# irfanICMLL/structure_knowledge_distillation

Hardware: AMD Instinct MI355X
Metric: distillation-step images/sec @512x512 (Pi+Pa+Ho) (higher is better)
Workload: dtype f32; 1 GPU; BASELINE configs[2]: ResNet18-PSPNet student + frozen ResNet101-PSPNet teacher, Pi+Pa+Ho (SAGAN D, spectral norm, WGAN-GP), batch 8 per GPU, 512x512, 19 classes; global_batch=8, parallelism=dp1

## Files before the change

structure_knowledge_distillation_amd/csrc/conv1x1.hip:

```cpp
#include <stdio.h>
#include <stdlib.h>

#include "conv_split_dev.hpp"

namespace skd {
namespace {

constexpr int kProMaxK = 512;

template <int TM>
struct Staging {
  float4 a[TM / kRPP], b[kRB];
};
struct ProParams {
  float4 pm, pi, pg, pb;
};

template <bool PRO, int TM>
__device__ __forceinline__ void stage_load(Staging<TM> &s, const float *__restrict__ X, const float *__restrict__ Wt, int k0,
                                           int gkq, const int64_t (&arow)[TM / kRPP], int64_t wrow0, int K) {
  const float *xa = X + k0 + gkq, *wb = Wt + k0 + gkq;
#pragma unroll
  for (int h = 0; h < TM / kRPP; ++h) s.a[h] = *reinterpret_cast<const float4 *>(xa + arow[h]);
#pragma unroll
  for (int h = 0; h < kRB; ++h) s.b[h] = *reinterpret_cast<const float4 *>(wb + wrow0 + (int64_t)(kRPP * h) * K);
}

__device__ __forceinline__ float pro_one(float x, float m, float is, float g, float b) {
  const float z = __builtin_fmaf((x - m) * is, g, b);
  return z < 0.f ? 0.f : z;
}

template <bool PRO, int TM>
__device__ __forceinline__ void stage_store(const Staging<TM> s, uint4 *stage, int srow, const float *ptab, int K, int kq) {
  constexpr int kRA = TM / kRPP;
  uint2 *sa = reinterpret_cast<uint2 *>(stage) + srow, *sb = reinterpret_cast<uint2 *>(stage + kOperandChunks) + srow;
  if (PRO) {
    ProParams pp;
    pp.pm = *reinterpret_cast<const float4 *>(ptab + kq);
    pp.pi = *reinterpret_cast<const float4 *>(ptab + K + kq);
    pp.pg = *reinterpret_cast<const float4 *>(ptab + 2 * K + kq);
    pp.pb = *reinterpret_cast<const float4 *>(ptab + 3 * K + kq);
#pragma unroll
    for (int h = 0; h < kRA; ++h) {
      float4 v = s.a[h];
      v.x = pro_one(v.x, pp.pm.x, pp.pi.x, pp.pg.x, pp.pb.x);
      v.y = pro_one(v.y, pp.pm.y, pp.pi.y, pp.pg.y, pp.pb.y);
      v.z = pro_one(v.z, pp.pm.z, pp.pi.z, pp.pg.z, pp.pb.z);
      v.w = pro_one(v.w, pp.pm.w, pp.pi.w, pp.pg.w, pp.pb.w);
      split_store(v, sa + 2 * kRPP * h);
    }
  } else {
#pragma unroll
    for (int h = 0; h < kRA; ++h) split_store(s.a[h], sa + 2 * kRPP * h);
  }
#pragma unroll
  for (int h = 0; h < kRB; ++h) split_store(s.b[h], sb + 2 * kRPP * h);
}

template <int TM, int ACT, bool HAS_RES, bool PRO, bool NT>
__device__ __forceinline__ void conv1x1_tile(const float *__restrict__ X, const float *__restrict__ Wt, const float *__restrict__ R,
                                             float *__restrict__ Y, const float *__restrict__ mean, const float *__restrict__ var,
                                             const float *__restrict__ weight, const float *__restrict__ bias,
                                             const float *__restrict__ ppack, float eps, float slope, int64_t M, int K, int N,
                                             int64_t m0, int n0, uint4 *lds) {
  constexpr int WM = TM / 64, kRA = TM / kRPP;
  f32x16 acc[WM][2];
#pragma unroll
  for (int i = 0; i < WM; ++i)
#pragma unroll
    for (int j = 0; j < 2; ++j)
#pragma unroll
      for (int q = 0; q < 16; ++q) acc[i][j][q] = 0.f;
  const int nk = K / kBK;
  const int gt = threadIdx.x, grow = gt / kQK, gkq = (gt % kQK) * 4;
  const int srow = plane_slot(grow, gkq);
  int64_t arow[kRA];
#pragma unroll
  for (int h = 0; h < kRA; ++h) {
    const int64_t m = m0 + grow + kRPP * h;
    arow[h] = (m > M - 1 ? M - 1 : m) * K;
  }
  const int64_t wrow0 = (int64_t)(n0 + grow) * K;
  float *ptab = reinterpret_cast<float *>(lds + 2 * kStageChunks);
  if (PRO) {
    for (int i = gt * 4; i < 4 * K; i += kThreads * 4) *reinterpret_cast<float4 *>(ptab + i) = *reinterpret_cast<const float4 *>(ppack + i);
    __syncthreads();
  }
  Staging<TM> st;
  stage_load<PRO, TM>(st, X, Wt, 0, gkq, arow, wrow0, K);
  stage_store<PRO, TM>(st, lds, srow, ptab, K, gkq);
  __syncthreads();
  int stage = 0;
  for (int kt = 0; kt < nk; ++kt) {
    const bool more = kt + 1 < nk;
    if (more) stage_load<PRO, TM>(st, X, Wt, (kt + 1) * kBK, gkq, arow, wrow0, K);
    tile_mma<TM>(lds + stage * kStageChunks, acc);
    if (more) stage_store<PRO, TM>(st, lds + (stage ^ 1) * kStageChunks, srow, ptab, K, (kt + 1) * kBK + gkq);
    __syncthreads();
    stage ^= 1;
  }
  const int lane = threadIdx.x & (kWave - 1), wid = threadIdx.x / kWave;
  const int wi = (wid >> 1) * (TM / 2), wj = (wid & 1) * 64;
  const bool full = m0 + TM <= M;
#pragma unroll
  for (int bj = 0; bj < 2; ++bj) {
    const int col = n0 + wj + bj * 32 + (lane & 31);
    const float mu = mean[col], is = inv_std_of(var[col], eps);
    const float ga = weight != nullptr ? fabsf(weight[col]) + eps : 1.f;
    const float be = bias != nullptr ? bias[col] : 0.f;
#pragma unroll
    for (int bi = 0; bi < WM; ++bi) {
      const int64_t row0 = m0 + wi + bi * 32;
      if (full)
        store_block<ACT, HAS_RES, true, NT>(acc[bi][bj], R, Y, row0, col, M, N, mu, is, ga, be, slope);
      else
        store_block<ACT, HAS_RES, false, NT>(acc[bi][bj], R, Y, row0, col, M, N, mu, is, ga, be, slope);
    }
  }
}

struct Geometry {
  int tiles_n, ct, pm;
  int64_t p_full, panels, grid;
  bool nt;
};
inline bool conv1x1_geometry(int64_t M, int K, int N, int cus, Geometry &g) {
  g.tiles_n = N / kTN;
  const int64_t tiles_m = cdiv(M, kTM);
  const int64_t tile_bytes = (int64_t)kTN * K * sizeof(float);
  g.ct = (int)((1 << 20) / tile_bytes);
  g.pm = (int)((2 << 20) / tile_bytes);
  if (g.ct < 1) g.ct = 1;
  if (g.pm < 1) g.pm = 1;
  g.nt = g.ct < g.tiles_n;
  if (!g.nt) { g.ct = g.tiles_n; g.pm = 1; }
  while (g.tiles_n % g.ct) --g.ct;
  g.p_full = g.panels = tiles_m;
  const int64_t slots = (int64_t)kMinWG * cus;
  const int64_t tiles = tiles_m * g.tiles_n;
  if (slots > 0 && tiles > slots && tiles % slots != 0) {
    g.p_full = (tiles / slots) * slots / g.tiles_n / 8 * 8;
    const int64_t rest_rows = M - g.p_full * kTM;
    g.panels = g.p_full + cdiv(rest_rows, kTM / 2);
  }
  const int64_t panels_per_xcd = cdiv(cdiv(g.panels, 8), g.pm) * g.pm;
  g.grid = panels_per_xcd * 8 * g.tiles_n;
  return g.grid <= 2147483647;
}

struct TileOf {
  int64_t m0;
  int rows, n0;
};
__host__ __device__ __forceinline__ TileOf conv1x1_tile_of(unsigned block, int64_t M, int tiles_n, int pm, int ct, int p_full) {
  const int xcd = block & 7, j = block >> 3;
  const int per_group = pm * tiles_n;
  const int group = j / per_group, r = j - group * per_group;
  const int per_chunk = pm * ct;
  const int chunk = r / per_chunk, r2 = r - chunk * per_chunk;
  const int pl = r2 / ct;
  const int tn = chunk * ct + (r2 - pl * ct);
  const int64_t tm = ((int64_t)group * pm + pl) * 8 + xcd;
  if (tn >= tiles_n) return TileOf{0, 0, 0};
  if (tm < p_full) {
    const int64_t m0 = tm * kTM;
    if (m0 >= M) return TileOf{0, 0, 0};
    return TileOf{m0, kTM, tn * kTN};
  }
  const int64_t m0 = (int64_t)p_full * kTM + (tm - p_full) * (kTM / 2);
  if (m0 >= M) return TileOf{0, 0, 0};
  return TileOf{m0, kTM / 2, tn * kTN};
}

template <int ACT, bool HAS_RES, bool PRO, bool NT>
__global__ __launch_bounds__(kThreads, kMinWG) void conv1x1_abn_kernel(
    const float *__restrict__ X, const float *__restrict__ Wt, const float *__restrict__ R, float *__restrict__ Y,
    const float *__restrict__ mean, const float *__restrict__ var, const float *__restrict__ weight,
    const float *__restrict__ bias, const float *__restrict__ ppack, float eps, float slope, int64_t M, int K, int N,
    int tiles_n, int pm, int ct, int p_full) {
  extern __shared__ __attribute__((aligned(16))) uint4 lds[];
  const TileOf t = conv1x1_tile_of(blockIdx.x, M, tiles_n, pm, ct, p_full);
  if (t.rows == kTM)
    conv1x1_tile<kTM, ACT, HAS_RES, PRO, NT>(X, Wt, R, Y, mean, var, weight, bias, ppack, eps, slope, M, K, N, t.m0, t.n0, lds);
  else if (t.rows == kTM / 2)
    conv1x1_tile<kTM / 2, ACT, HAS_RES, PRO, NT>(X, Wt, R, Y, mean, var, weight, bias, ppack, eps, slope, M, K, N, t.m0, t.n0, lds);
}

__global__ void pack_eval_params_kernel(int K, const float *__restrict__ mean, const float *__restrict__ var,
                                        const float *__restrict__ weight, const float *__restrict__ bias, float eps,
                                        float *__restrict__ pack) {
  const int k = blockIdx.x * blockDim.x + threadIdx.x;
  if (k >= K) return;
  pack[k] = mean[k];
  pack[K + k] = inv_std_of(var[k], eps);
  pack[2 * (int64_t)K + k] = weight != nullptr ? fabsf(weight[k]) + eps : 1.f;
  pack[3 * (int64_t)K + k] = bias != nullptr ? bias[k] : 0.f;
}

template <int ACT, bool HAS_RES, bool PRO, bool NT = false>
static int launch(const float *X, const float *Wt, const float *R, float *Y, const float *mean, const float *var,
                  const float *weight, const float *bias, const float *ppack, float eps, float slope, int64_t M, int K, int N,
                  hipStream_t st) {
  static PerDeviceFlag ready;
  bool *rdy = ready.get();
  if (rdy == nullptr) return 0;
  if (!*rdy) {
    if (hipFuncSetAttribute(reinterpret_cast<const void *>(conv1x1_abn_kernel<ACT, HAS_RES, PRO, NT>),
                            hipFuncAttributeMaxDynamicSharedMemorySize, (int)(kConvLds + sizeof(float) * 4 * kProMaxK)) != hipSuccess) return 0;
    *rdy = true;
  }
  const size_t lds_bytes = kConvLds + (PRO ? sizeof(float) * 4 * (size_t)K : 0);
  Geometry g;
  if (!conv1x1_geometry(M, K, N, cu_count(st), g)) return 0;
  if (g.nt && !NT) return launch<ACT, HAS_RES, PRO, true>(X, Wt, R, Y, mean, var, weight, bias, ppack, eps, slope, M, K, N, st);
  conv1x1_abn_kernel<ACT, HAS_RES, PRO, NT><<<dim3((unsigned)g.grid), dim3(kThreads), lds_bytes, st>>>(
      X, Wt, R, Y, mean, var, weight, bias, ppack, eps, slope, M, K, N, g.tiles_n, g.pm, g.ct, (int)g.p_full);
  return ok();
}

}
}

using namespace skd;

extern "C" {

int skd_conv1x1_abn_supported(int64_t M, int K, int N) { return M > 0 && K > 0 && N > 0 && K % kBK == 0 && N % kTN == 0; }

int skd_conv1x1_abn_geometry(int64_t M, int K, int N, int cus, int64_t *out) {
  Geometry g;
  if (!skd_conv1x1_abn_supported(M, K, N) || cus < 0 || !out || !conv1x1_geometry(M, K, N, cus, g)) return 0;
  out[0] = g.tiles_n; out[1] = g.ct; out[2] = g.pm; out[3] = g.p_full; out[4] = g.panels; out[5] = g.grid; out[6] = g.nt;
  return 1;
}

int skd_conv1x1_abn_tile_of(int64_t M, int K, int N, int cus, int64_t block, int64_t count, int64_t *out) {
  Geometry g;
  if (!skd_conv1x1_abn_supported(M, K, N) || cus < 0 || !out || !conv1x1_geometry(M, K, N, cus, g)) return 0;
  if (block < 0 || count < 0 || block > g.grid || count > g.grid - block) return 0;
  for (int64_t i = 0; i < count; ++i) {
    const TileOf t = conv1x1_tile_of((unsigned)(block + i), M, g.tiles_n, g.pm, g.ct, (int)g.p_full);
    out[3 * i] = t.m0; out[3 * i + 1] = t.rows; out[3 * i + 2] = t.n0;
  }
  return 1;
}

static int conv1x1_dispatch(int64_t M, int K, int N, const float *x, const float *w, const float *residual, float *out,
                            const float *mean, const float *var, const float *weight, const float *bias, const float *ppack,
                            float eps, int activation, float slope, skd_stream_t stream) {
  if (!skd_conv1x1_abn_supported(M, K, N) || !x || !w || !out || !mean || !var) return 0;
  if ((reinterpret_cast<uintptr_t>(x) | reinterpret_cast<uintptr_t>(w) | reinterpret_cast<uintptr_t>(ppack)) & 15) return 0;
  hipStream_t st = as_stream(stream);
#define SKD_C11(A)                                                                                                        \
  if (ppack != nullptr)                                                                                                   \
    return residual ? launch<A, true, true>(x, w, residual, out, mean, var, weight, bias, ppack, eps, slope, M, K, N, st)   \
                    : launch<A, false, true>(x, w, residual, out, mean, var, weight, bias, ppack, eps, slope, M, K, N, st); \
  return residual ? launch<A, true, false>(x, w, residual, out, mean, var, weight, bias, nullptr, eps, slope, M, K, N, st) \
                  : launch<A, false, false>(x, w, residual, out, mean, var, weight, bias, nullptr, eps, slope, M, K, N, st)
  switch (activation) {
    case SKD_ACT_NONE: SKD_C11(SKD_ACT_NONE);
    case SKD_ACT_RELU: SKD_C11(SKD_ACT_RELU);
    case SKD_ACT_LEAKY_RELU: SKD_C11(SKD_ACT_LEAKY_RELU);
    default: return 0;
  }
#undef SKD_C11
}

int skd_conv1x1_abn_nhwc(int64_t M, int K, int N, const float *x, const float *w, const float *residual, float *out,
                         const float *mean, const float *var, const float *weight, const float *bias, float eps,
                         int activation, float slope, skd_stream_t stream) {
  return conv1x1_dispatch(M, K, N, x, w, residual, out, mean, var, weight, bias, nullptr, eps, activation, slope, stream);
}

int skd_abn_pack_eval_params(int K, const float *mean, const float *var, const float *weight, const float *bias, float eps,
                             float *pack, skd_stream_t stream) {
  if (K <= 0 || !mean || !var || !pack) return 0;
  pack_eval_params_kernel<<<dim3((unsigned)cdiv(K, 256)), dim3(256), 0, as_stream(stream)>>>(K, mean, var, weight, bias, eps, pack);
  return ok();
}

int skd_conv1x1_abn_pro_nhwc(int64_t M, int K, int N, const float *x, const float *w, const float *residual, float *out,
                             const float *mean, const float *var, const float *weight, const float *bias, float eps,
                             const float *ppack, int activation, float slope, skd_stream_t stream) {
  if (!ppack || K > kProMaxK) return 0;
  return conv1x1_dispatch(M, K, N, x, w, residual, out, mean, var, weight, bias, ppack, eps, activation, slope, stream);
}

}
```

structure_knowledge_distillation_amd/csrc/conv3x3.hip:

```cpp
#include "conv_split_dev.hpp"

namespace skd {
namespace {

constexpr int kTileChunks = kOperandChunks;
constexpr int kBChunksPerThread = kTileChunks / kThreads;

template <int TM>
struct Staging3 {
  float4 a[TM / kRPP];
  uint4 b[kBChunksPerThread];
};

struct TapCursor {
  int tap, c0;
  int64_t shift;
};

__device__ __forceinline__ int64_t tap_shift(int tap, int W, int dil, int Cin) {
  const int ty = tap / 3, tx = tap - 3 * ty;
  return ((int64_t)(ty - 1) * W + (tx - 1)) * dil * Cin;
}

template <int TM>
__device__ __forceinline__ void stage_load3(Staging3<TM> &s, const float *__restrict__ X, const uint4 *__restrict__ bsrc,
                                            const TapCursor &cur, const int64_t (&abase)[TM / kRPP], const unsigned (&mask)[TM / kRPP]) {
#pragma unroll
  for (int h = 0; h < TM / kRPP; ++h) {
    s.a[h] = make_float4(0.f, 0.f, 0.f, 0.f);
    if ((mask[h] >> cur.tap) & 1u) s.a[h] = *reinterpret_cast<const float4 *>(X + abase[h] + cur.shift + cur.c0);
  }
#pragma unroll
  for (int p = 0; p < kBChunksPerThread; ++p) s.b[p] = bsrc[p * kPlaneChunks];
}

template <int TM>
__device__ __forceinline__ void stage_store3(const Staging3<TM> s, uint4 *stage, int srow) {
  uint2 *sa = reinterpret_cast<uint2 *>(stage) + srow;
#pragma unroll
  for (int h = 0; h < TM / kRPP; ++h) split_store(s.a[h], sa + 2 * kRPP * h);
  uint4 *sb = stage + kOperandChunks + threadIdx.x;
#pragma unroll
  for (int p = 0; p < kBChunksPerThread; ++p) sb[p * kPlaneChunks] = s.b[p];
}

template <int TM, int ACT>
__device__ __forceinline__ void conv3x3_tile(const float *__restrict__ X, const uint4 *__restrict__ Bp, float *__restrict__ Y,
                                             const float *__restrict__ cbias, const float *__restrict__ mean,
                                             const float *__restrict__ var, const float *__restrict__ weight,
                                             const float *__restrict__ bias, float eps, float slope, int64_t M, int H, int W,
                                             int Cin, int N, int dil, int64_t m0, int tn, uint4 *lds) {
  constexpr int WM = TM / 64, kRA = TM / kRPP;
  f32x16 acc[WM][2], low[WM][2];
#pragma unroll
  for (int i = 0; i < WM; ++i)
#pragma unroll
    for (int j = 0; j < 2; ++j)
#pragma unroll
      for (int q = 0; q < 16; ++q) acc[i][j][q] = low[i][j][q] = 0.f;
  const int nk = 9 * (Cin / kBK);
  const int gt = threadIdx.x, grow = gt / kQK, gkq = (gt % kQK) * 4;
  const int srow = plane_slot(grow, gkq);
  int64_t abase[kRA];
  unsigned mask[kRA];
  const int64_t hw = (int64_t)H * W;
#pragma unroll
  for (int h = 0; h < kRA; ++h) {
    const int64_t m = m0 + grow + kRPP * h;
    const bool live = m < M;
    const int64_t mm = live ? m : 0;
    const int pix = (int)(mm % hw);
    const int py = pix / W, px = pix - py * W;
    unsigned bits = 0;
#pragma unroll
    for (int tap = 0; tap < 9; ++tap) {
      const int64_t y = py + (int64_t)(tap / 3 - 1) * dil, x = px + (int64_t)(tap % 3 - 1) * dil;
      if (live && y >= 0 && y < H && x >= 0 && x < W) bits |= 1u << tap;
    }
    mask[h] = bits;
    abase[h] = mm * Cin + gkq;
  }
  const uint4 *bsrc = Bp + (int64_t)tn * nk * kTileChunks + gt;
  TapCursor cur = {0, 0, tap_shift(0, W, dil, Cin)};
  Staging3<TM> st;
  stage_load3<TM>(st, X, bsrc, cur, abase, mask);
  stage_store3<TM>(st, lds, srow);
  __syncthreads();
  int stage = 0;
  for (int kt = 0; kt < nk; ++kt) {
    const bool more = kt + 1 < nk;
    if (more) {
      cur.c0 += kBK;
      if (cur.c0 == Cin) {
        cur.c0 = 0;
        ++cur.tap;
        cur.shift = tap_shift(cur.tap, W, dil, Cin);
      }
      stage_load3<TM>(st, X, bsrc + (int64_t)(kt + 1) * kTileChunks, cur, abase, mask);
    }
    tile_mma<TM>(lds + stage * kStageChunks, low, acc);
    if (more) stage_store3<TM>(st, lds + (stage ^ 1) * kStageChunks, srow);
    __syncthreads();
    stage ^= 1;
  }
  const int lane = threadIdx.x & (kWave - 1), wid = threadIdx.x / kWave;
  const int wi = (wid >> 1) * (TM / 2), wj = (wid & 1) * 64;
  const bool full = m0 + TM <= M;
#pragma unroll
  for (int bj = 0; bj < 2; ++bj) {
    const int col = tn * kTN + wj + bj * 32 + (lane & 31);
    const bool bn = mean != nullptr;
    const float mu = bn ? mean[col] : 0.f, is = bn ? inv_std_of(var[col], eps) : 1.f;
    const float ga = bn && weight != nullptr ? fabsf(weight[col]) + eps : 1.f;
    const float be = bn && bias != nullptr ? bias[col] : 0.f;
    const float cb = cbias != nullptr ? cbias[col] : 0.f;
#pragma unroll
    for (int bi = 0; bi < WM; ++bi) {
#pragma unroll
      for (int q = 0; q < 16; ++q) acc[bi][bj][q] += low[bi][bj][q];
      if (cbias != nullptr) {
#pragma unroll
        for (int q = 0; q < 16; ++q) acc[bi][bj][q] += cb;
      }
      const int64_t row0 = m0 + wi + bi * 32;
      if (full)
        store_block<ACT, false, true, false>(acc[bi][bj], nullptr, Y, row0, col, M, N, mu, is, ga, be, slope);
      else
        store_block<ACT, false, false, false>(acc[bi][bj], nullptr, Y, row0, col, M, N, mu, is, ga, be, slope);
    }
  }
}

template <int ACT, bool TALL>
__global__ __launch_bounds__(kThreads, TALL ? 2 : kMinWG) __attribute__((amdgpu_waves_per_eu(TALL ? 2 : kMinWG, TALL ? 2 : kMinWG)))
void conv3x3_split_kernel(
    const float *__restrict__ X, const uint4 *__restrict__ Bp, float *__restrict__ Y, const float *__restrict__ cbias,
    const float *__restrict__ mean, const float *__restrict__ var, const float *__restrict__ weight,
    const float *__restrict__ bias, float eps, float slope, int64_t M, int H, int W, int Cin, int N, int dil, int tiles_n,
    int p_full) {
  extern __shared__ __attribute__((aligned(16))) uint4 lds[];
  const int xcd = blockIdx.x & 7, j = blockIdx.x >> 3;
  const int pl = j / tiles_n, tn = j - pl * tiles_n;
  const int64_t tm = (int64_t)pl * 8 + xcd;
  if (TALL && tm < p_full) {
    const int64_t m0 = tm * kTM;
    if (m0 >= M) return;
    conv3x3_tile<kTM, ACT>(X, Bp, Y, cbias, mean, var, weight, bias, eps, slope, M, H, W, Cin, N, dil, m0, tn, lds);
  } else {
    const int64_t m0 = (int64_t)p_full * kTM + (tm - p_full) * (kTM / 2);
    if (m0 >= M) return;
    conv3x3_tile<kTM / 2, ACT>(X, Bp, Y, cbias, mean, var, weight, bias, eps, slope, M, H, W, Cin, N, dil, m0, tn, lds);
  }
}

__global__ void conv3x3_pack_kernel(const float *__restrict__ Wt, int64_t sn, int64_t sc, int64_t sy, int64_t sx, int Cin, int nk,
                                    int64_t chunks, uint4 *__restrict__ pack) {
  const int64_t idx = (int64_t)blockIdx.x * blockDim.x + threadIdx.x;
  if (idx >= chunks) return;
  const int chunk = (int)(idx % kPlaneChunks);
  const int64_t tile = idx / kPlaneChunks;
  const int kt = (int)(tile % nk), tn = (int)(tile / nk);
  const int kh = chunk >> 7, row = (chunk & 127) ^ (kh * 4);
  const int k0 = kt * kBK + kh * 8, tap = k0 / Cin, c0 = k0 - tap * Cin;
  const int ty = tap / 3, tx = tap - 3 * ty;
  const float *src = Wt + (int64_t)(tn * kTN + row) * sn + ty * sy + tx * sx;
  float v[8];
#pragma unroll
  for (int i = 0; i < 8; ++i) v[i] = src[(c0 + i) * sc];
  uint2 lo[3], hi[3];
  split4(make_float4(v[0], v[1], v[2], v[3]), lo[0], lo[1], lo[2]);
  split4(make_float4(v[4], v[5], v[6], v[7]), hi[0], hi[1], hi[2]);
#pragma unroll
  for (int p = 0; p < 3; ++p) pack[(tile * 3 + p) * kPlaneChunks + chunk] = make_uint4(lo[p].x, lo[p].y, hi[p].x, hi[p].y);
}

template <int ACT, bool TALL>
static int launch3(const float *X, const uint4 *Bp, float *Y, const float *cbias, const float *mean, const float *var,
                   const float *weight, const float *bias, float eps, float slope, int64_t M, int H, int W, int Cin, int N, int dil,
                   int geometry, hipStream_t st) {
  static PerDeviceFlag ready;
  bool *rdy = ready.get();
  if (rdy == nullptr) return 0;
  if (!*rdy) {
    if (hipFuncSetAttribute(reinterpret_cast<const void *>(conv3x3_split_kernel<ACT, TALL>),
                            hipFuncAttributeMaxDynamicSharedMemorySize, (int)kConvLds) != hipSuccess) return 0;
    *rdy = true;
  }
  const int tiles_n = N / kTN;
  const int64_t tiles_m = cdiv(M, kTM);
  int64_t p_full = TALL ? tiles_m : 0;
  if (TALL && geometry == 3) {
    const int64_t slots = 2 * (int64_t)cu_count(st), tiles = tiles_m * tiles_n;
    if (slots > 0 && tiles % slots != 0) p_full = (tiles / slots) * slots / tiles_n / 8 * 8;
  }
  const int64_t panels = p_full < tiles_m ? p_full + cdiv(M - p_full * kTM, kTM / 2) : tiles_m;
  const int64_t grid = cdiv(panels, 8) * 8 * tiles_n;
  if (grid > 2147483647) return 0;
  conv3x3_split_kernel<ACT, TALL><<<dim3((unsigned)grid), dim3(kThreads), kConvLds, st>>>(
      X, Bp, Y, cbias, mean, var, weight, bias, eps, slope, M, H, W, Cin, N, dil, tiles_n, (int)p_full);
  return ok();
}

template <int ACT>
static int launch3g(const float *X, const uint4 *Bp, float *Y, const float *cbias, const float *mean, const float *var,
                    const float *weight, const float *bias, float eps, float slope, int64_t M, int H, int W, int Cin, int N, int dil,
                    int geometry, hipStream_t st) {
  if (geometry == 0) geometry = cdiv(M, kTM) * (N / kTN) > 2 * (int64_t)cu_count(st) ? 3 : 2;
  if (geometry == 1 || geometry == 3)
    return launch3<ACT, true>(X, Bp, Y, cbias, mean, var, weight, bias, eps, slope, M, H, W, Cin, N, dil, geometry, st);
  return launch3<ACT, false>(X, Bp, Y, cbias, mean, var, weight, bias, eps, slope, M, H, W, Cin, N, dil, geometry, st);
}

}
}

using namespace skd;

extern "C" {

int skd_conv3x3_split_supported(int Cin, int Cout, int stride, int padding, int dilation, int groups) {
  return Cin > 0 && Cout > 0 && Cin % kBK == 0 && Cout % kTN == 0 && stride == 1 && dilation >= 1 && padding == dilation && groups == 1;
}

int64_t skd_conv3x3_split_pack_bytes(int Cin, int Cout) {
  if (!skd_conv3x3_split_supported(Cin, Cout, 1, 1, 1, 1)) return 0;
  return (int64_t)(Cout / kTN) * (9 * (Cin / kBK)) * kTileChunks * (int64_t)sizeof(uint4);
}

int skd_conv3x3_split_pack_weights(int Cin, int Cout, const float *w, int64_t stride_n, int64_t stride_c, int64_t stride_y,
                                   int64_t stride_x, void *pack, int64_t pack_bytes, skd_stream_t stream) {
  const int64_t need = skd_conv3x3_split_pack_bytes(Cin, Cout);
  if (need == 0 || !w || !pack || pack_bytes < need || (reinterpret_cast<uintptr_t>(pack) & 15)) return 0;
  if (stride_n < 0 || stride_c < 0 || stride_y < 0 || stride_x < 0) return 0;
  const int nk = 9 * (Cin / kBK);
  const int64_t chunks = (int64_t)(Cout / kTN) * nk * kPlaneChunks;
  conv3x3_pack_kernel<<<dim3((unsigned)cdiv(chunks, 256)), dim3(256), 0, as_stream(stream)>>>(
      w, stride_n, stride_c, stride_y, stride_x, Cin, nk, chunks, static_cast<uint4 *>(pack));
  return ok();
}

int skd_conv3x3_split_nhwc(int B, int H, int W, int Cin, int Cout, int dilation, const float *x, const void *wpack, float *out,
                           const float *conv_bias, const float *mean, const float *var, const float *weight, const float *bias,
                           float eps, int activation, float slope, int geometry, skd_stream_t stream) {
  if (!skd_conv3x3_split_supported(Cin, Cout, 1, dilation, dilation, 1) || B < 1 || H < 1 || W < 1) return 0;
  if (!x || !wpack || !out || (mean == nullptr) != (var == nullptr) || geometry < 0 || geometry > 3) return 0;
  if ((reinterpret_cast<uintptr_t>(x) | reinterpret_cast<uintptr_t>(wpack)) & 15) return 0;
  if ((int64_t)H * W > 2147483647 || dilation > (1 << 24)) return 0;
  const int64_t M = (int64_t)B * H * W;
  hipStream_t st = as_stream(stream);
  const uint4 *bp = static_cast<const uint4 *>(wpack);
  switch (activation) {
    case SKD_ACT_NONE: return launch3g<SKD_ACT_NONE>(x, bp, out, conv_bias, mean, var, weight, bias, eps, slope, M, H, W, Cin, Cout, dilation, geometry, st);
    case SKD_ACT_RELU: return launch3g<SKD_ACT_RELU>(x, bp, out, conv_bias, mean, var, weight, bias, eps, slope, M, H, W, Cin, Cout, dilation, geometry, st);
    case SKD_ACT_LEAKY_RELU: return launch3g<SKD_ACT_LEAKY_RELU>(x, bp, out, conv_bias, mean, var, weight, bias, eps, slope, M, H, W, Cin, Cout, dilation, geometry, st);
    default: return 0;
  }
}

}
```

structure_knowledge_distillation_amd/csrc/conv_split_dev.hpp:

```cpp
#pragma once
#include <atomic>

#include "skd_common.hpp"

namespace skd {

typedef float f32x16 __attribute__((ext_vector_type(16)));
typedef __bf16 bf16x8 __attribute__((ext_vector_type(8)));
typedef __bf16 bf16x2 __attribute__((ext_vector_type(2)));
typedef float f32x2 __attribute__((ext_vector_type(2)));

constexpr int kTM = 128, kTN = 128, kBK = 16, kMinWG = 3;
constexpr int kQK = kBK / 4;
constexpr int kRPP = kThreads / kQK;
constexpr int kRB = kTN / kRPP;
constexpr int kPlaneChunks = 2 * 128;
constexpr int kOperandChunks = 3 * kPlaneChunks;
constexpr int kStageChunks = 2 * kOperandChunks;
constexpr size_t kConvLds = sizeof(uint4) * 2 * kStageChunks;

__device__ __forceinline__ float inv_std_of(float var, float eps) { return (var != 0.f || eps != 0.f) ? 1.f / sqrtf(var + eps) : 0.f; }

__device__ __forceinline__ uint32_t pack_bf16(float x, float y) {
  const f32x2 v = {x, y};
  return __builtin_bit_cast(uint32_t, __builtin_convertvector(v, bf16x2));
}
__device__ __forceinline__ float bf16_lo(uint32_t u) { return __uint_as_float(u << 16); }
__device__ __forceinline__ float bf16_hi(uint32_t u) { return __uint_as_float(u & 0xffff0000u); }

__device__ __forceinline__ void split4(float4 v, uint2 &p0, uint2 &p1, uint2 &p2) {
  p0.x = pack_bf16(v.x, v.y);
  p0.y = pack_bf16(v.z, v.w);
  v.x -= bf16_lo(p0.x); v.y -= bf16_hi(p0.x); v.z -= bf16_lo(p0.y); v.w -= bf16_hi(p0.y);
  p1.x = pack_bf16(v.x, v.y);
  p1.y = pack_bf16(v.z, v.w);
  v.x -= bf16_lo(p1.x); v.y -= bf16_hi(p1.x); v.z -= bf16_lo(p1.y); v.w -= bf16_hi(p1.y);
  p2.x = pack_bf16(v.x, v.y);
  p2.y = pack_bf16(v.z, v.w);
}
__device__ __forceinline__ void split_store(float4 v, uint2 *dst) {
  uint2 p0, p1, p2;
  split4(v, p0, p1, p2);
  dst[0] = p0;
  dst[2 * kPlaneChunks] = p1;
  dst[4 * kPlaneChunks] = p2;
}

__device__ __forceinline__ int plane_slot(int row, int gkq) {
  const int kh = gkq >> 3;
  return 2 * (kh * 128 + (row ^ (kh * 4))) + ((gkq >> 2) & 1);
}

template <int TM>
__device__ __forceinline__ void tile_mma(const uint4 *stage, f32x16 (&lo)[TM / 64][2], f32x16 (&hi)[TM / 64][2]) {
  constexpr int WM = TM / 64;
  const int lane = threadIdx.x & (kWave - 1), wid = threadIdx.x / kWave;
  const int wi = (wid >> 1) * (TM / 2), wj = (wid & 1) * 64;
  const int half = lane >> 5, r = lane & 31;
  const uint4 *pa = stage + half * 128 + ((wi + r) ^ (half * 4));
  const uint4 *pb = stage + kOperandChunks + half * 128 + ((wj + r) ^ (half * 4));
  bf16x8 a[WM][3], b[2][3];
#pragma unroll
  for (int p = 0; p < 3; ++p) {
#pragma unroll
    for (int i = 0; i < WM; ++i) a[i][p] = __builtin_bit_cast(bf16x8, pa[p * kPlaneChunks + 32 * i]);
#pragma unroll
    for (int j = 0; j < 2; ++j) b[j][p] = __builtin_bit_cast(bf16x8, pb[p * kPlaneChunks + 32 * j]);
  }
  constexpr int kPA[6] = {0, 1, 2, 0, 1, 0}, kPB[6] = {2, 1, 0, 1, 0, 0};
#pragma unroll
  for (int t = 0; t < 6; ++t)
#pragma unroll
    for (int i = 0; i < WM; ++i)
#pragma unroll
      for (int j = 0; j < 2; ++j) {
        f32x16 &dst = t < 5 ? lo[i][j] : hi[i][j];
        dst = __builtin_amdgcn_mfma_f32_32x32x16_bf16(a[i][kPA[t]], b[j][kPB[t]], dst, 0, 0, 0);
      }
}
template <int TM>
__device__ __forceinline__ void tile_mma(const uint4 *stage, f32x16 (&acc)[TM / 64][2]) { tile_mma<TM>(stage, acc, acc); }

template <int ACT, bool HAS_RES, bool FULL, bool NT>
__device__ __forceinline__ void store_block(const f32x16 &acc, const float *__restrict__ R, float *__restrict__ Y, int64_t row0,
                                            int col, int64_t M, int N, float mu, float is, float ga, float be, float slope) {
  const int lane = threadIdx.x & (kWave - 1);
  float rv[16];
  int64_t off[16];
#pragma unroll
  for (int q = 0; q < 16; ++q) {
    const int64_t row = row0 + (q & 3) + 8 * (q >> 2) + 4 * (lane >> 5);
    off[q] = row * N + col;
    rv[q] = 0.f;
    if (HAS_RES && (FULL || row < M)) rv[q] = NT ? __builtin_nontemporal_load(R + off[q]) : R[off[q]];
  }
#pragma unroll
  for (int q = 0; q < 16; ++q) {
    const int64_t row = row0 + (q & 3) + 8 * (q >> 2) + 4 * (lane >> 5);
    float z = ((acc[q] - mu) * is) * ga + be;
    if (HAS_RES) z += rv[q];
    if (ACT == SKD_ACT_RELU) z = z < 0.f ? 0.f : z;
    if (ACT == SKD_ACT_LEAKY_RELU) z = z < 0.f ? z * slope : z;
    if (FULL || row < M) {
      if (NT) __builtin_nontemporal_store(z, Y + off[q]);
      else Y[off[q]] = z;
    }
  }
}

inline int cu_count(hipStream_t st) {
  static std::atomic<int> cus[64];
  int dev = -1;
  if (hipStreamGetDevice(st, &dev) != hipSuccess) {
    (void)hipGetLastError();
    if (hipGetDevice(&dev) != hipSuccess) return 0;
  }
  if (dev < 0 || dev >= 64) return 0;
  int n = cus[dev].load(std::memory_order_relaxed);
  if (n == 0 && hipDeviceGetAttribute(&n, hipDeviceAttributeMultiprocessorCount, dev) == hipSuccess && n > 0)
    cus[dev].store(n, std::memory_order_relaxed);
  return n > 0 ? n : 0;
}

}
```

Measured before the change: 144.2 images/sec.

## Add two-deep register prefetch k-loop shared by 1x1 and 3x3 conv kernels

Replaces the single-stage register staging loops in the 1x1 and 3x3 split-bf16 MFMA conv kernels with a shared templated k_loop. The loop keeps two register staging buffers, loads tile kt+2 from global memory while tile kt+1 is written to LDS and tile kt is multiplied, and is unrolled by two with a peeled tail. The goal is to hide more global-load latency behind MFMA work. In exchange it doubles the staging registers, which could lower occupancy or cause spills.

```diff
diff --git a/structure_knowledge_distillation_amd/csrc/conv1x1.hip b/structure_knowledge_distillation_amd/csrc/conv1x1.hip
--- a/structure_knowledge_distillation_amd/csrc/conv1x1.hip
+++ b/structure_knowledge_distillation_amd/csrc/conv1x1.hip
@@ -7,6 +7,8 @@
 namespace {
 
 constexpr int kProMaxK = 512;
+
+constexpr int kDepth1x1 = 2;
 
 template <int TM>
 struct Staging {
@@ -32,7 +34,7 @@
 }
 
 template <bool PRO, int TM>
-__device__ __forceinline__ void stage_store(const Staging<TM> s, uint4 *stage, int srow, const float *ptab, int K, int kq) {
+__device__ __forceinline__ void stage_store(const Staging<TM> &s, uint4 *stage, int srow, const float *ptab, int K, int kq) {
   constexpr int kRA = TM / kRPP;
   uint2 *sa = reinterpret_cast<uint2 *>(stage) + srow, *sb = reinterpret_cast<uint2 *>(stage + kOperandChunks) + srow;
   if (PRO) {
@@ -58,6 +60,21 @@
   for (int h = 0; h < kRB; ++h) split_store(s.b[h], sb + 2 * kRPP * h);
 }
 
+template <bool PRO, int TM>
+struct Tile1 {
+  typedef Staging<TM> Stg;
+  const float *__restrict__ X, *__restrict__ Wt;
+  const float *ptab;
+  int K, gkq, srow;
+  int64_t wrow0, arow[TM / kRPP];
+  f32x16 (&acc)[TM / 64][2];
+  __device__ __forceinline__ void load(Stg &s, int kt) const { stage_load<PRO, TM>(s, X, Wt, kt * kBK, gkq, arow, wrow0, K); }
+  __device__ __forceinline__ void store(const Stg &s, uint4 *stage, int kt) const {
+    stage_store<PRO, TM>(s, stage, srow, ptab, K, kt * kBK + gkq);
+  }
+  __device__ __forceinline__ void mma(const uint4 *stage) const { tile_mma<TM>(stage, acc); }
+};
+
 template <int TM, int ACT, bool HAS_RES, bool PRO, bool NT>
 __device__ __forceinline__ void conv1x1_tile(const float *__restrict__ X, const float *__restrict__ Wt, const float *__restrict__ R,
                                              float *__restrict__ Y, const float *__restrict__ mean, const float *__restrict__ var,
@@ -87,19 +104,10 @@
     for (int i = gt * 4; i < 4 * K; i += kThreads * 4) *reinterpret_cast<float4 *>(ptab + i) = *reinterpret_cast<const float4 *>(ppack + i);
     __syncthreads();
   }
-  Staging<TM> st;
-  stage_load<PRO, TM>(st, X, Wt, 0, gkq, arow, wrow0, K);
-  stage_store<PRO, TM>(st, lds, srow, ptab, K, gkq);
-  __syncthreads();
-  int stage = 0;
-  for (int kt = 0; kt < nk; ++kt) {
-    const bool more = kt + 1 < nk;
-    if (more) stage_load<PRO, TM>(st, X, Wt, (kt + 1) * kBK, gkq, arow, wrow0, K);
-    tile_mma<TM>(lds + stage * kStageChunks, acc);
-    if (more) stage_store<PRO, TM>(st, lds + (stage ^ 1) * kStageChunks, srow, ptab, K, (kt + 1) * kBK + gkq);
-    __syncthreads();
-    stage ^= 1;
-  }
+  Tile1<PRO, TM> tile = {X, Wt, ptab, K, gkq, srow, wrow0, {}, acc};
+#pragma unroll
+  for (int h = 0; h < kRA; ++h) tile.arow[h] = arow[h];
+  k_loop<kDepth1x1>(tile, nk, lds);
   const int lane = threadIdx.x & (kWave - 1), wid = threadIdx.x / kWave;
   const int wi = (wid >> 1) * (TM / 2), wj = (wid & 1) * 64;
   const bool full = m0 + TM <= M;
diff --git a/structure_knowledge_distillation_amd/csrc/conv3x3.hip b/structure_knowledge_distillation_amd/csrc/conv3x3.hip
--- a/structure_knowledge_distillation_amd/csrc/conv3x3.hip
+++ b/structure_knowledge_distillation_amd/csrc/conv3x3.hip
@@ -5,6 +5,7 @@
 
 constexpr int kTileChunks = kOperandChunks;
 constexpr int kBChunksPerThread = kTileChunks / kThreads;
+constexpr int kDepth3x3 = 2;
 
 template <int TM>
 struct Staging3 {
@@ -23,19 +24,22 @@
 }
 
 template <int TM>
-__device__ __forceinline__ void stage_load3(Staging3<TM> &s, const float *__restrict__ X, const uint4 *__restrict__ bsrc,
-                                            const TapCursor &cur, const int64_t (&abase)[TM / kRPP], const unsigned (&mask)[TM / kRPP]) {
+__device__ __forceinline__ void stage_load3_b(Staging3<TM> &s, const uint4 *__restrict__ bsrc) {
+#pragma unroll
+  for (int p = 0; p < kBChunksPerThread; ++p) s.b[p] = bsrc[p * kPlaneChunks];
+}
+template <int TM>
+__device__ __forceinline__ void stage_load3_a(Staging3<TM> &s, const float *__restrict__ X, const TapCursor &cur,
+                                              const int64_t (&abase)[TM / kRPP], const unsigned (&mask)[TM / kRPP]) {
 #pragma unroll
   for (int h = 0; h < TM / kRPP; ++h) {
     s.a[h] = make_float4(0.f, 0.f, 0.f, 0.f);
     if ((mask[h] >> cur.tap) & 1u) s.a[h] = *reinterpret_cast<const float4 *>(X + abase[h] + cur.shift + cur.c0);
   }
-#pragma unroll
-  for (int p = 0; p < kBChunksPerThread; ++p) s.b[p] = bsrc[p * kPlaneChunks];
-}
-
-template <int TM>
-__device__ __forceinline__ void stage_store3(const Staging3<TM> s, uint4 *stage, int srow) {
+}
+
+template <int TM>
+__device__ __forceinline__ void stage_store3(const Staging3<TM> &s, uint4 *stage, int srow) {
   uint2 *sa = reinterpret_cast<uint2 *>(stage) + srow;
 #pragma unroll
   for (int h = 0; h < TM / kRPP; ++h) split_store(s.a[h], sa + 2 * kRPP * h);
@@ -43,6 +47,30 @@
 #pragma unroll
   for (int p = 0; p < kBChunksPerThread; ++p) sb[p * kPlaneChunks] = s.b[p];
 }
+
+template <int TM>
+struct Tile3 {
+  typedef Staging3<TM> Stg;
+  const float *__restrict__ X;
+  const uint4 *__restrict__ bsrc;
+  int srow, W, dil, Cin;
+  TapCursor cur;
+  int64_t abase[TM / kRPP];
+  unsigned mask[TM / kRPP];
+  f32x16 (&low)[TM / 64][2], (&acc)[TM / 64][2];
+  __device__ __forceinline__ void load(Stg &s, int kt) {
+    stage_load3_a<TM>(s, X, cur, abase, mask);
+    stage_load3_b<TM>(s, bsrc + (int64_t)kt * kTileChunks);
+    cur.c0 += kBK;
+    if (cur.c0 == Cin) {
+      cur.c0 = 0;
+      ++cur.tap;
+      cur.shift = tap_shift(cur.tap, W, dil, Cin);
+    }
+  }
+  __device__ __forceinline__ void store(const Stg &s, uint4 *stage, int) const { stage_store3<TM>(s, stage, srow); }
+  __device__ __forceinline__ void mma(const uint4 *stage) const { tile_mma<TM>(stage, low, acc); }
+};
 
 template <int TM, int ACT>
 __device__ __forceinline__ void conv3x3_tile(const float *__restrict__ X, const uint4 *__restrict__ Bp, float *__restrict__ Y,
@@ -81,28 +109,13 @@
     abase[h] = mm * Cin + gkq;
   }
   const uint4 *bsrc = Bp + (int64_t)tn * nk * kTileChunks + gt;
-  TapCursor cur = {0, 0, tap_shift(0, W, dil, Cin)};
-  Staging3<TM> st;
-  stage_load3<TM>(st, X, bsrc, cur, abase, mask);
-  stage_store3<TM>(st, lds, srow);
-  __syncthreads();
-  int stage = 0;
-  for (int kt = 0; kt < nk; ++kt) {
-    const bool more = kt + 1 < nk;
-    if (more) {
-      cur.c0 += kBK;
-      if (cur.c0 == Cin) {
-        cur.c0 = 0;
-        ++cur.tap;
-        cur.shift = tap_shift(cur.tap, W, dil, Cin);
-      }
-      stage_load3<TM>(st, X, bsrc + (int64_t)(kt + 1) * kTileChunks, cur, abase, mask);
-    }
-    tile_mma<TM>(lds + stage * kStageChunks, low, acc);
-    if (more) stage_store3<TM>(st, lds + (stage ^ 1) * kStageChunks, srow);
-    __syncthreads();
-    stage ^= 1;
-  }
+  Tile3<TM> tile = {X, bsrc, srow, W, dil, Cin, {0, 0, tap_shift(0, W, dil, Cin)}, {}, {}, low, acc};
+#pragma unroll
+  for (int h = 0; h < kRA; ++h) {
+    tile.abase[h] = abase[h];
+    tile.mask[h] = mask[h];
+  }
+  k_loop<kDepth3x3>(tile, nk, lds);
   const int lane = threadIdx.x & (kWave - 1), wid = threadIdx.x / kWave;
   const int wi = (wid >> 1) * (TM / 2), wj = (wid & 1) * 64;
   const bool full = m0 + TM <= M;
diff --git a/structure_knowledge_distillation_amd/csrc/conv_split_dev.hpp b/structure_knowledge_distillation_amd/csrc/conv_split_dev.hpp
--- a/structure_knowledge_distillation_amd/csrc/conv_split_dev.hpp
+++ b/structure_knowledge_distillation_amd/csrc/conv_split_dev.hpp
@@ -81,6 +81,39 @@
 template <int TM>
 __device__ __forceinline__ void tile_mma(const uint4 *stage, f32x16 (&acc)[TM / 64][2]) { tile_mma<TM>(stage, acc, acc); }
 
+template <int DEPTH, bool STEADY, class Tile>
+__device__ __forceinline__ void k_trip(Tile &t, typename Tile::Stg &fill, typename Tile::Stg &next, const uint4 *cur, uint4 *nxt,
+                                       int kt, int nk) {
+  static_assert(DEPTH == 1 || DEPTH == 2, "load look-ahead of one or two K-tiles");
+  if (DEPTH == 2) {
+    if (STEADY || kt + 2 < nk) t.load(fill, kt + 2);
+    if (STEADY || kt + 1 < nk) t.store(next, nxt, kt + 1);
+    t.mma(cur);
+  } else {
+    if (STEADY || kt + 1 < nk) t.load(next, kt + 1);
+    t.mma(cur);
+    if (STEADY || kt + 1 < nk) t.store(next, nxt, kt + 1);
+  }
+  __syncthreads();
+}
+template <int DEPTH, class Tile>
+__device__ __forceinline__ void k_loop(Tile &t, int nk, uint4 *lds) {
+  typename Tile::Stg s0, s1;
+  uint4 *const l0 = lds, *const l1 = lds + kStageChunks;
+  t.load(s0, 0);
+  if (DEPTH == 2 && nk > 1) t.load(s1, 1);
+  t.store(s0, l0, 0);
+  __syncthreads();
+  int kt = 0;
+  for (; kt + 3 < nk; kt += 2) {
+    k_trip<DEPTH, true>(t, s0, s1, l0, l1, kt, nk);
+    k_trip<DEPTH, true>(t, s1, s0, l1, l0, kt + 1, nk);
+  }
+  k_trip<DEPTH, false>(t, s0, s1, l0, l1, kt, nk);
+  if (kt + 1 < nk) k_trip<DEPTH, false>(t, s1, s0, l1, l0, kt + 1, nk);
+  if (kt + 2 < nk) k_trip<DEPTH, false>(t, s0, s1, l0, l1, kt + 2, nk);
+}
+
 template <int ACT, bool HAS_RES, bool FULL, bool NT>
 __device__ __forceinline__ void store_block(const f32x16 &acc, const float *__restrict__ R, float *__restrict__ Y, int64_t row0,
                                             int col, int64_t M, int N, float mu, float is, float ga, float be, float slope) {
```

Result: faster. 147.9 images/sec (median of 6 runs) (+2.5%).
